# rehakvoj1/BIH-GPU-Raytracer

Measured on NVIDIA B200. Metric: Mrays/s, higher is better.
Workload: dtype f32

## Files before the change

### bih-gpu-raytracer_b200/csrc/api.cu

```cuda
#include "bihrt_internal.cuh"
#include <algorithm>
#include <cstdarg>
#include <cstdio>
#include <cstdlib>
#include <cstring>
#include <vector>

int bihrt_fail(bihrt_ctx* c, int code, const char* fmt, ...) {
    char buf[512];
    va_list ap;
    va_start(ap, fmt);
    vsnprintf(buf, sizeof buf, fmt, ap);
    va_end(ap);
    if (c) c->err = buf;
    return code;
}

#define ENTER(c) do { if (!(c)) return BIHRT_ERR_INVALID; BIHRT_CUDA((c), cudaSetDevice((c)->device)); } while (0)

static bool is_device_ptr(const void* p) {
    cudaPointerAttributes at;
    if (cudaPointerGetAttributes(&at, p) != cudaSuccess) { cudaGetLastError(); return false; }
    return at.type == cudaMemoryTypeDevice || at.type == cudaMemoryTypeManaged;
}
// ... 58 lines not shown
        size_t P = 256;
        while (P < (size_t)cap) P <<= 1;
        if ((rc = dev_alloc(c, &c->d_heaps, 4 * P))) return rc;
    }
    return BIHRT_OK;
}

extern "C" {

int bihrt_version(void) { return BIHRT_VERSION; }

int bihrt_create(bihrt_ctx** out, const bihrt_config* cfg) {
    if (!out) return BIHRT_ERR_INVALID;
    *out = nullptr;
    int ndev = 0;
    if (cudaGetDeviceCount(&ndev) != cudaSuccess || ndev == 0) { cudaGetLastError(); return BIHRT_ERR_CUDA; }
    bihrt_ctx* c = new (std::nothrow) bihrt_ctx();
    if (!c) return BIHRT_ERR_NOMEM;
    c->device = cfg ? cfg->device : 0;
    if (c->device < 0 || c->device >= ndev) { delete c; return BIHRT_ERR_INVALID; }
    cudaDeviceProp prop;
    if (cudaSetDevice(c->device) != cudaSuccess || cudaGetDeviceProperties(&prop, c->device) != cudaSuccess) { delete c; return BIHRT_ERR_CUDA; }
    if (prop.major < 10) { delete c; return BIHRT_ERR_CUDA; }
    c->sm_count = prop.multiProcessorCount;
    if (cudaStreamCreateWithFlags(&c->own_stream, cudaStreamNonBlocking) != cudaSuccess) { delete c; return BIHRT_ERR_CUDA; }
    c->stream = c->own_stream;
    cudaEventCreate(&c->ev0); cudaEventCreate(&c->ev1);
    int rc = 0;
    rc |= dev_alloc(c, &c->d_hist, 4096);
    rc |= dev_alloc(c, &c->d_scenebox_enc, 24);
    rc |= dev_alloc(c, &c->d_counters, 8);
    rc |= dev_alloc(c, &c->d_work, 1024);
    if (cudaHostAlloc((void**)&c->h_status, 64, cudaHostAllocMapped | cudaHostAllocPortable) != cudaSuccess ||
        cudaHostGetDevicePointer((void**)&c->d_status_map, c->h_status, 0) != cudaSuccess) { cudaGetLastError(); rc |= 1; }
    else *c->h_status = 0;
    if (rc) { bihrt_destroy(c); return BIHRT_ERR_NOMEM; }
    if (bihrt_build_setup(c) != BIHRT_OK) { bihrt_destroy(c); return BIHRT_ERR_CUDA; }
    *out = c;
    return BIHRT_OK;
}

void bihrt_destroy(bihrt_ctx* c) {
    if (!c) return;
    cudaSetDevice(c->device);
    cudaDeviceSynchronize();
    dev_free(&c->d_tri_in); dev_free(&c->d_blob);
    for (int i = 0; i < 2; i++) { dev_free(&c->d_keys[i]); dev_free(&c->d_vals[i]); }
    dev_free(&c->d_umc); dev_free(&c->d_first); dev_free(&c->d_hist); dev_free(&c->d_lookback);
    dev_free(&c->d_heaps); dev_free(&c->d_scenebox_enc);
    dev_free(&c->d_keys64[0]); dev_free(&c->d_keys64[1]); dev_free(&c->d_lookback_q);
    dev_free(&c->d_fb); dev_free(&c->d_counters); dev_free(&c->d_work);
    dev_free(&c->d_wtab); dev_free(&c->d_wscratch);
    for (auto& ts : c->tile_slots) { dev_free(&ts.cost); dev_free(&ts.order); }
    if (c->d_io) { cudaFree(c->d_io); c->d_io = nullptr; }
    for (int i = 0; i < 2; i++) { dev_free(&c->d_rs_keys[i]); dev_free(&c->d_rs_vals[i]); }
    dev_free(&c->d_rs_hist); dev_free(&c->d_rs_lookback); dev_free(&c->d_rs_hdr);
    if (c->h_status) { cudaFreeHost(c->h_status); c->h_status = nullptr; }
    if (c->ev0) cudaEventDestroy(c->ev0);
    if (c->ev1) cudaEventDestroy(c->ev1);
    if (c->build_graph_exec) cudaGraphExecDestroy(c->build_graph_exec);
    for (int i = 0; i < BIHRT_PROF_EVENTS; i++) if (c->prof_ev[i]) cudaEventDestroy(c->prof_ev[i]);
    if (c->own_stream) cudaStreamDestroy(c->own_stream);
    delete c;
}

const char* bihrt_last_error(const bihrt_ctx* c) { return c ? c->err.c_str() : "null context"; }

int bihrt_set_stream(bihrt_ctx* c, void* s) {
    ENTER(c);
    BIHRT_CUDA(c, cudaStreamSynchronize(c->stream));
    c->stream = (s == BIHRT_STREAM_OWN) ? c->own_stream : (cudaStream_t)s;
    return BIHRT_OK;
}

int bihrt_get_stream(bihrt_ctx* c, void** s) {
    if (!c || !s) return BIHRT_ERR_INVALID;
    *s = (void*)c->stream;
    return BIHRT_OK;
}

static int check_status(bihrt_ctx* c) {
    const uint32_t st = c->h_status ? *(volatile uint32_t*)c->h_status : 0u;
    if (st & 0x100u) return bihrt_fail(c, BIHRT_ERR_STATE, "the BIH in this context is a %s tree but the context traces %s trees: set the option morton_bits "
                                       "to the builder's value before adopting a replicated BIH", c->built_quality ? "parity" : "quality-mode", c->built_quality ? "quality-mode" : "parity");
    if (st) return bihrt_fail(c, BIHRT_ERR_INTERNAL, "device watchdog tripped during build (status %u): the BIH is invalid, rebuild", st);
    return BIHRT_OK;
}

int bihrt_sync(bihrt_ctx* c) {
    ENTER(c);
    BIHRT_CUDA(c, cudaStreamSynchronize(c->stream));
    return check_status(c);
}

int bihrt_set_option(bihrt_ctx* c, const char* name, int64_t v) {
    if (!c || !name) return BIHRT_ERR_INVALID;
    if (!strcmp(name, "trace_blocks_per_sm")) c->opt_trace_blocks_per_sm = (int)v;
    else if (!strcmp(name, "build_graph")) c->opt_build_graph = (int)v;
    else if (!strcmp(name, "morton_bits")) {
        if (v != 30 && v != 63) return bihrt_fail(c, BIHRT_ERR_INVALID, "morton_bits must be 30 (reference grid) or 63 (quality mode)");
        c->opt_morton_bits = (int)v;
        if (c->build_graph_exec) { cudaGraphExecDestroy(c->build_graph_exec); c->build_graph_exec = nullptr; }
    }
    else if (!strcmp(name, "leaf_cap")) {
        if (v < 1 || v > 64) return bihrt_fail(c, BIHRT_ERR_INVALID, "leaf_cap must be 1..64");
        c->opt_leaf_cap = (int)v;
        if (c->build_graph_exec) { cudaGraphExecDestroy(c->build_graph_exec); c->build_graph_exec = nullptr; }
    }
    else if (!strcmp(name, "debug_trip_watchdog")) {
        c->opt_debug_trip_watchdog = (int)v;
        if (c->build_graph_exec) { cudaGraphExecDestroy(c->build_graph_exec); c->build_graph_exec = nullptr; }
    }
    else if (!strcmp(name, "profile")) {
        BIHRT_CUDA(c, cudaSetDevice(c->device));
        c->opt_profile = (int)v;
        if (v) for (int i = 0; i < BIHRT_PROF_EVENTS; i++) if (!c->prof_ev[i]) cudaEventCreate(&c->prof_ev[i]);
    }
    else if (!strcmp(name, "trace_lane_groups")) c->opt_lane_groups = (int)v;
    else if (!strcmp(name, "trace_sort_rays")) c->opt_sort_rays = (int)v;
    else if (!strcmp(name, "trace_sm_queues")) c->opt_sm_queues = (int)v;
    else if (!strcmp(name, "trace_tile_sort_below")) c->opt_tile_sort_below = v;
    else if (!strcmp(name, "trace_tile_order")) { c->opt_tile_order = (int)v; for (auto& ts : c->tile_slots) ts.valid = false; }
    else if (!strcmp(name, "interleave_chunk")) c->opt_interleave_chunk = (int)std::max<int64_t>(1, std::min<int64_t>(1024, v));
    else return bihrt_fail(c, BIHRT_ERR_INVALID, "unknown option '%s'", name);
    return BIHRT_OK;
}

int bihrt_get_stat(bihrt_ctx* c, const char* name, int64_t* v) {
    if (!c || !name || !v) return BIHRT_ERR_INVALID;
    if (!strcmp(name, "kernel_launches")) *v = c->kernel_launches;
    else if (!strcmp(name, "sm_count")) *v = c->sm_count;
    else if (!strcmp(name, "trace_warp_node_steps") || !strcmp(name, "trace_warp_leaf_steps")) {
        unsigned long long h[2];
        BIHRT_CUDA(c, cudaSetDevice(c->device));
        BIHRT_CUDA(c, cudaMemcpyAsync(h, c->d_counters + 4, 16, cudaMemcpyDeviceToHost, c->stream));
        BIHRT_CUDA(c, cudaStreamSynchronize(c->stream));
        *v = (int64_t)h[name[11] == 'n' ? 0 : 1];
    }
    else if (!strncmp(name, "build_stage_ns_", 15)) {
        const int i = atoi(name + 15);
        if (!c->opt_profile || i < 0 || i + 1 >= c->prof_count) return bihrt_fail(c, BIHRT_ERR_STATE, "no profile for stage %d (set option profile=1 and build)", i);
        BIHRT_CUDA(c, cudaEventSynchronize(c->prof_ev[i + 1]));
        float ms = 0;
        BIHRT_CUDA(c, cudaEventElapsedTime(&ms, c->prof_ev[i], c->prof_ev[i + 1]));
        *v = (int64_t)(ms * 1e6f);
    }
    else return bihrt_fail(c, BIHRT_ERR_INVALID, "unknown stat '%s'", name);
    return BIHRT_OK;
}

static int upload_triangles(bihrt_ctx* c, const float* xyz9, int64_t n) {
    if (n > 0) {
        cudaMemcpyKind kind = is_device_ptr(xyz9) ? cudaMemcpyDeviceToDevice : cudaMemcpyHostToDevice;
        BIHRT_CUDA(c, cudaMemcpyAsync(c->d_tri_in, xyz9, (size_t)n * 36, kind, c->stream));
    }
    return BIHRT_OK;
}

int bihrt_scene_load_triangles(bihrt_ctx* c, const float* xyz9, int64_t n) {
    ENTER(c);
    if (n < 0 || (n > 0 && !xyz9)) return bihrt_fail(c, BIHRT_ERR_INVALID, "bad triangle array");
    if (n >= BIH_MAX_TRIS) return bihrt_fail(c, BIHRT_ERR_INVALID, "at most 2^29-1 triangles (29-bit child references)");
    int rc = ensure_capacity(c, n, true);
    if (rc) return rc;
    if (n != c->n) {
        bind_blob(c, std::max<int64_t>(n, 1));
        if (c->build_graph_exec) { cudaGraphExecDestroy(c->build_graph_exec); c->build_graph_exec = nullptr; }
    }
    c->n = n; c->have_scene = true; c->built = false; c->topology_valid = false;
    return upload_triangles(c, xyz9, n);
}

int bihrt_scene_update_vertices(bihrt_ctx* c, const float* xyz9, int64_t n) {
    ENTER(c);
    if (!c->have_scene || !c->d_tri_in) return bihrt_fail(c, BIHRT_ERR_STATE, "no scene loaded");
    if (n != c->n) return bihrt_fail(c, BIHRT_ERR_INVALID, "update must keep the triangle count (%lld != %lld)", (long long)n, (long long)c->n);
    c->built = false;
    return upload_triangles(c, xyz9, n);
}

int bihrt_scene_load_obj(bihrt_ctx* c, const char* path) {
    ENTER(c);
    if (!path) return BIHRT_ERR_INVALID;
    FILE* f = fopen(path, "r");
    if (!f) return bihrt_fail(c, BIHRT_ERR_IO, "cannot open '%s'", path);
    std::vector<float> verts, tris;
    std::vector<long> poly;
    char line[4096];
    int rc = BIHRT_OK;
    while (fgets(line, sizeof line, f)) {
// ... 715 lines not shown
```

### bih-gpu-raytracer_b200/csrc/bihrt_internal.cuh

```cuda
#pragma once
#include <cuda_runtime.h>
#include <stdint.h>
#include <string>
#include "../../include/bihrt.h"

struct __align__(16) BihNode {
    float    clip0;
    float    clip1;
    uint32_t ref_l;
    uint32_t ref_r;
    float    lbox[6];
    float    rbox[6];
};
static_assert(sizeof(BihNode) == 64, "node is one 64-byte record");
#define BIH_REF_LEAF  0x80000000u
#define BIH_REF_NODE(idx, axis) (((uint32_t)(idx) << 2) | (uint32_t)(axis))
#define BIH_REF_LEAFREF(slot)   (BIH_REF_LEAF | ((uint32_t)(slot) << 2))
#define BIH_REF_INDEX(ref)      (((ref) & 0x7FFFFFFFu) >> 2)
#define BIH_REF_AXIS(ref)       ((ref) & 3u)
#define BIH_MAX_TRIS  (1ll << 29)

struct __align__(16) BihTri {
    float    v0x, v0y, v0z, e1x;
    float    e1y, e1z, e2x, e2y;
// ... 18 lines not shown
#define BIHRT_PROF_EVENTS 16
struct bihrt_group;
struct bihrt_ctx {
    bihrt_group* group = nullptr; int group_rank = 0;
    int          device = 0;
    cudaStream_t stream = nullptr;
    cudaStream_t own_stream = nullptr;
    std::string  err;
    int          sm_count = 148;

    float*   d_tri_in = nullptr;
    int64_t  n = 0, cap_n = 0;
    bool     have_scene = false, built = false;
    bool     topology_valid = false;

    uint8_t* d_blob = nullptr;
    size_t   blob_cap = 0;
    BihHeader* d_hdr = nullptr;
    BihNode*   d_nodes = nullptr;
    BihTri*    d_tris = nullptr;

    uint32_t *d_keys[2] = {nullptr, nullptr}, *d_vals[2] = {nullptr, nullptr};
    uint64_t *d_keys64[2] = {nullptr, nullptr};
    uint32_t *d_lookback_q = nullptr; size_t lookback_q_words = 0;
    uint32_t *d_umc = nullptr;
    uint32_t *d_first = nullptr;
    uint32_t *d_hist = nullptr;
    uint32_t *d_lookback = nullptr;
    size_t    lookback_words = 0;
    float4   *d_heaps = nullptr;
    uint32_t *d_scenebox_enc = nullptr;

    uint32_t* d_fb = nullptr; int fb_w = 0, fb_h = 0; size_t fb_cap = 0;
    bool      fb_exported = false;
    uint32_t* h_status = nullptr;
    uint32_t* d_status_map = nullptr;
    void*     d_io = nullptr; size_t io_cap = 0;
    unsigned long long* d_counters = nullptr;
    uint32_t *d_rs_keys[2] = {nullptr, nullptr}, *d_rs_vals[2] = {nullptr, nullptr}, *d_rs_hist = nullptr, *d_rs_lookback = nullptr;
    BihHeader* d_rs_hdr = nullptr; size_t rs_cap = 0;
    int opt_sort_rays = 0;
    uint32_t* d_work = nullptr;
    struct TileKey {
        int mode = -1, w = 0, h = 0, gshift = 0, nsamp = 0, shard_index = 0, shard_count = 0, il_index = 0, il_count = 0, il_cshift = 0;
        int64_t nrays = 0; uint32_t ntiles = 0;
        bool operator==(const TileKey& o) const {
            return mode == o.mode && w == o.w && h == o.h && gshift == o.gshift && nsamp == o.nsamp && shard_index == o.shard_index &&
                   shard_count == o.shard_count && il_index == o.il_index && il_count == o.il_count && il_cshift == o.il_cshift &&
                   nrays == o.nrays && ntiles == o.ntiles;
        }
    };
    struct TileSlot { TileKey key; bool valid = false; uint32_t *cost = nullptr, *order = nullptr; size_t cap = 0; };
    TileSlot tile_slots[4]; int tile_next = 0;

    cudaEvent_t ev0 = nullptr, ev1 = nullptr;
    bool        build_timed = false;

    int opt_trace_blocks_per_sm = 0;
    int opt_lane_groups = -1;
    int opt_interleave_chunk = 8;
    int opt_tile_order = 1;
    int64_t opt_tile_sort_below = 4 << 20;
    int opt_sm_queues = -1;
    int64_t kernel_launches = 0;
    int opt_build_graph = 1;
    cudaGraphExec_t build_graph_exec = nullptr; int64_t build_graph_n = -1, build_graph_launches = 0;
    int opt_morton_bits = 30;
    int opt_leaf_cap = 4;
    bool built_quality = false;
    float*    d_wtab = nullptr; int64_t wtab_slots = 0;
    uint32_t* d_wscratch = nullptr;
    bool      wtab_valid = false;
    int opt_debug_trip_watchdog = 0;
    int opt_profile = 0;
    cudaEvent_t prof_ev[BIHRT_PROF_EVENTS] = {};
    int prof_count = 0;
};

int  bihrt_fail(bihrt_ctx* c, int code, const char* fmt, ...);
#define BIHRT_CUDA(c, call) do { cudaError_t e_ = (call); if (e_ != cudaSuccess) \
    return bihrt_fail((c), BIHRT_ERR_CUDA, "%s failed: %s (%s:%d)", #call, cudaGetErrorString(e_), __FILE__, __LINE__); } while (0)

#define H_HIST      0
#define H_TILECTR   2048
#define H_WORDS     2064
#define SORT_TILE   4096

int bihrt_sort_pairs_launch(bihrt_ctx* c, uint32_t* keys[2], uint32_t* vals[2], uint32_t n, int passes, uint32_t* hist, uint32_t* lookback, BihHeader* hdr);
int bihrt_build_launch(bihrt_ctx* c);
int bihrt_build_setup(bihrt_ctx* c);
int bihrt_build_launch_q(bihrt_ctx* c);
int bihrt_refit_launch(bihrt_ctx* c);
#define STACK_DEPTH_PARITY  32
#define STACK_DEPTH_QUALITY 96
struct TraceArgs {
    const BihHeader* hdr; const BihNode* nodes; const BihTri* tris;
    const bihrt_ray* rays; int64_t nrays;
    const uint32_t* perm;
    int any_hit; float tmax;
    float* out_t; int32_t* out_slot; int32_t* out_prim;
    bihrt_camera cam; int w, h, spp; uint64_t seed; uint32_t flags; int shard_index, shard_count;
    int s_begin, s_end;
    int il_index, il_count;
    int il_cshift;
    const uint32_t* tile_order;
    uint32_t* tile_cost;
    int gshift;
    uint32_t* fb;
    unsigned long long* counters; uint32_t* work;
    uint32_t* status_map;
    int queues;
    const bihrt_ray_interval* rays_iv;
    float* out_u; float* out_v; float* out_ng;
};
int bihrt_trace_launch(bihrt_ctx* c, const TraceArgs& a, int mode , bool counted);
int bihrt_resolve_launch(bihrt_ctx* c, uint32_t* fb, int npix, int spp);
int bihrt_tile_order_launch(bihrt_ctx* c, uint32_t* cost, uint32_t* order, uint32_t ntiles, bool full_sort);
struct ClosestArgs {
    const BihHeader* hdr; const BihNode* nodes; const BihTri* tris;
    const bihrt_point_query* pts; int64_t n;
    float* out_d2; float* out_u; float* out_v; int32_t* out_slot; int32_t* out_prim; float* out_q; float* out_ng;
    uint32_t* work;
    uint32_t* status_map;
};
int bihrt_closest_launch(bihrt_ctx* c, const ClosestArgs& a);
#define WTAB_FLOATS 32
#define WTAB_SCRATCH_WORDS(n) (4 * (size_t)(n) + 16)
struct WindingArgs {
    const BihHeader* hdr; const BihNode* nodes; const BihTri* tris;
    const float* wtab;
    const bihrt_point_query* pts; int64_t n;
    float b2;
    float* out_w;
    uint32_t* work;
    uint32_t* status_map;
};
int bihrt_winding_table_launch(bihrt_ctx* c);
int bihrt_winding_launch(bihrt_ctx* c, const WindingArgs& a);
int bihrt_ray_sort_launch(bihrt_ctx* c, const bihrt_ray* rays, int64_t n, const uint32_t** perm);
int bihrt_secondary_launch(bihrt_ctx* c, const float* t, const int32_t* slot, int64_t n, uint32_t* tile_cnt, unsigned long long* total,
                           const bihrt_camera& cam, int w, int h, int spp, uint64_t seed, uint32_t flags, int kind, const float light[3],
                           bihrt_ray* out_rays, int32_t* out_sample);

#ifdef __CUDACC__
__device__ __forceinline__ uint32_t enc_float(float f) {
    uint32_t u = __float_as_uint(f);
    return (u & 0x80000000u) ? ~u : (u | 0x80000000u);
}
__device__ __forceinline__ float dec_float(uint32_t u) {
    return __uint_as_float((u & 0x80000000u) ? (u & 0x7FFFFFFFu) : ~u);
}

__host__ __device__ __forceinline__ uint32_t bihrt_mix32(uint32_t x) {
    x ^= x >> 16; x *= 0x7feb352du; x ^= x >> 15; x *= 0x846ca68bu; x ^= x >> 16;
    return x;
}
__device__ __forceinline__ float bihrt_jitter(uint64_t seed, uint32_t pixel, uint32_t sample, uint32_t dim) {
    uint32_t h = bihrt_mix32((uint32_t)seed ^ bihrt_mix32(pixel + 0x9e3779b9u * (sample * 2u + dim + 1u)) ^ (uint32_t)(seed >> 32));
    return __fmul_rn((float)((h >> 8) + 1u), 1.0f / 16777216.0f);
// ... 10 lines not shown
```

### bih-gpu-raytracer_b200/csrc/trace.cu

```cuda
#include "bihrt_internal.cuh"
#include <float.h>

#define FULL 0xffffffffu
#define NONE 0xFFFFFFFFu
#define TRACE_THREADS 128
#define TRACE_MIN_BLOCKS 8
constexpr int NODE_STEPS = 4;

#define OCT_MIXED 8
#define BOX_EPS 2.384185791015625e-07f

#define DET_EPS __uint_as_float(0x358637beu)

struct Hit { float t; int slot; };

__device__ __forceinline__ float fmin3(float a, float b, float c) { float r; asm("min.f32 %0, %1, %2, %3;" : "=f"(r) : "f"(a), "f"(b), "f"(c)); return r; }
__device__ __forceinline__ float fmax3(float a, float b, float c) { float r; asm("max.f32 %0, %1, %2, %3;" : "=f"(r) : "f"(a), "f"(b), "f"(c)); return r; }

__device__ __forceinline__ uint32_t pack_colour(uint32_t hits, int samples) {
    const float fh = (float)hits, fm = (float)(samples - (int)hits), fs = (float)samples;
    float cr = __fdiv_rn(__fadd_rn(__fmul_rn(fh, 255.f), __fmul_rn(fm, 20.f)), fs);
    float cb = __fdiv_rn(__fmul_rn(fm, 40.f), fs);
    cr = fmaxf(0.f, fminf(255.f, cr));
    cb = fmaxf(0.f, fminf(255.f, cb));
// ... 10 lines not shown
__device__ __forceinline__ float mt_u(float ox, float oy, float oz, const float4& q0, float px, float py, float pz, float inv,
                                      float& tx, float& ty, float& tz) {
    tx = __fsub_rn(ox, q0.x); ty = __fsub_rn(oy, q0.y); tz = __fsub_rn(oz, q0.z);
    return __fmul_rn(__fadd_rn(__fadd_rn(__fmul_rn(tx, px), __fmul_rn(ty, py)), __fmul_rn(tz, pz)), inv);
}
__device__ __forceinline__ float mt_v(float dx, float dy, float dz, float e1x, float e1y, float e1z, float tx, float ty, float tz, float inv,
                                      float& qx, float& qy, float& qz) {
    qx = __fsub_rn(__fmul_rn(ty, e1z), __fmul_rn(e1y, tz));
    qy = __fsub_rn(__fmul_rn(tz, e1x), __fmul_rn(e1z, tx));
    qz = __fsub_rn(__fmul_rn(tx, e1y), __fmul_rn(e1x, ty));
    return __fmul_rn(__fadd_rn(__fadd_rn(__fmul_rn(dx, qx), __fmul_rn(dy, qy)), __fmul_rn(dz, qz)), inv);
}

template <bool COUNTED, bool FIRST, bool RANGE = false, bool TWO_SIDED = false>
__device__ __forceinline__ void test_leaf(const char* __restrict__ first_tri, float ox, float oy, float oz,
                                          float dx, float dy, float dz, Hit& h, uint32_t& ntris, uint32_t& wleaf,
                                          const float* tlo_p = nullptr) {
    const float4* p = reinterpret_cast<const float4*>(first_tri);
    for (;;) {
        const float4 q0 = __ldg(p), q1 = __ldg(p + 1), q2 = __ldg(p + 2);
        if (COUNTED) { ntris++; const uint32_t am = __activemask(); wleaf += ((threadIdx.x & 31) == __ffs(am) - 1); }
        const float e1x = q0.w, e1y = q1.x, e1z = q1.y, e2x = q1.z, e2y = q1.w, e2z = q2.x;
        float px, py, pz;
        const float det = mt_det(dx, dy, dz, e1x, e1y, e1z, e2x, e2y, e2z, px, py, pz);
        if (!((TWO_SIDED ? fabsf(det) : det) < DET_EPS)) {
            const float inv = __frcp_rn(det);
            float tx, ty, tz;
            const float u = mt_u(ox, oy, oz, q0, px, py, pz, inv, tx, ty, tz);
            if (!(u < 0.f || u > 1.f)) {
                float qx, qy, qz;
                const float v = mt_v(dx, dy, dz, e1x, e1y, e1z, tx, ty, tz, inv, qx, qy, qz);
                if (!(v < 0.f || __fadd_rn(u, v) > 1.f)) {
                    const float t = __fmul_rn(__fadd_rn(__fadd_rn(__fmul_rn(e2x, qx), __fmul_rn(e2y, qy)), __fmul_rn(e2z, qz)), inv);
                    if (t > (RANGE ? *tlo_p : 0.f) && t < h.t) {
                        h.t = t; h.slot = (int)__float_as_uint(q2.w);
                        if (FIRST) break;
                    }
                }
            }
        }
        if (__float_as_uint(q2.z) & 1u) break;
        p += 3;
    }
}

template <int MODE, bool COUNTED, bool Q>
__global__ void __launch_bounds__(TRACE_THREADS, TRACE_MIN_BLOCKS) k_trace(TraceArgs a) {
    constexpr int STACK_DEPTH = Q ? STACK_DEPTH_QUALITY : STACK_DEPTH_PARITY;
    constexpr bool COVER = MODE == 1;
    constexpr bool OCTS = MODE == 1;
    constexpr bool LIST = MODE == 0 || MODE == 3 || MODE == 4;
    constexpr bool RANGE = MODE == 3 || MODE == 4;
    constexpr bool TWO_SIDED = MODE == 4;
    __shared__ __align__(16) float s_ray[TRACE_THREADS * 10];
    const int lane = threadIdx.x & 31;
    const uint32_t lt = (1u << lane) - 1u;
    float* my_ray = s_ray + threadIdx.x * 10;
    const char* __restrict__ nodes_b = reinterpret_cast<const char*>(a.nodes);
    const char* __restrict__ tris_b = reinterpret_cast<const char*>(a.tris);
    const BihTri* __restrict__ tris = a.tris;
    const uint32_t nu = a.hdr->nu;
    if (a.hdr->status != 0) return;
    if ((a.hdr->quality != 0) != Q) {
        if (blockIdx.x == 0 && threadIdx.x == 0 && a.status_map) *a.status_map = 0x100u;
        return;
    }
    const float blo[3] = { a.hdr->lo[0], a.hdr->lo[1], a.hdr->lo[2] }, bhi[3] = { a.hdr->hi[0], a.hdr->hi[1], a.hdr->hi[2] };
    uint32_t nnodes = 0, ntris = 0, maxsp = 0;
    uint32_t wnode = 0, wleaf = 0;

    uint64_t total;
    int tx = 1;
    if (LIST) total = a.tile_cost ? (((uint64_t)a.nrays + 1023u) >> 10) << 10 : (uint64_t)a.nrays;
    else {
        tx = (a.w + 31) / 32;
        const int ty = (a.h + 31) / 32, T = tx * ty;
        const int my_tiles = T > a.shard_index ? (T - a.shard_index + a.shard_count - 1) / a.shard_count : 0;
        total = ((uint64_t)my_tiles * 1024u) << a.gshift;
    }
    const int gshift = LIST ? 0 : a.gshift;
    const int nsamp = LIST ? 1 : ((a.s_end - a.s_begin) >> gshift);
    uint32_t my_queue = 0;
    if (a.queues > 1) { asm("mov.u32 %0, %%smid;" : "=r"(my_queue)); my_queue %= (uint32_t)a.queues; }
    uint64_t pool_next = 0, pool_end = 0;
    long long unit_t0 = 0; uint32_t unit_tile = 0xFFFFFFFFu;
    bool exhausted = false;

    uint64_t item = ~0ull;
    int s = 0, s0 = 0;
    uint32_t hits = 0, pixel = 0, pxy = 0;
    float ix = 1.f, iy = 1.f, iz = 1.f, nx = 0.f, ny = 0.f, nz = 0.f, bpad = 0.f;
    uint32_t cur = NONE;
    float rMin = 0.f, pMin = 0.f, pMax = 0.f;
    Hit h; h.t = FLT_MAX; h.slot = -1;
    bool tracing = false;
    uint4 stack[STACK_DEPTH];
    int sp = 0;
#define STACK_RESET() do { sp = 0; } while (0)
#define STACK_PUSH(item) do { stack[sp] = (item); sp++; } while (0)
#define STACK_POP(e) do { sp--; (e) = stack[sp]; } while (0)
    const uint32_t root_ref = BIH_REF_NODE(0, a.hdr->root_axis);
    const bool direct = MODE == 1 && gshift > 0 && !(a.flags & BIHRT_RENDER_COUNTS);
    const uint32_t ray_smem = (uint32_t)__cvta_generic_to_shared(my_ray);

    for (;;) {
        const uint32_t busy = ~__ballot_sync(FULL, cur == NONE);
        if (busy == 0) {
            bool want_item = false, finishing = false;
            if (cur == NONE) {
                if (tracing) {
                    tracing = false;
                    if (MODE == 1) hits += (h.slot >= 0);
                    else if (RANGE) {
                        const bool hit = h.slot >= 0;
                        const bool rec = a.out_u || a.out_v || a.out_ng;
                        float u = 0.f, v = 0.f, gx = 0.f, gy = 0.f, gz = 0.f;
                        int32_t prim = -1;
                        if (hit && (rec || a.out_prim)) {
                            const float4* tq = reinterpret_cast<const float4*>(tris + h.slot);
                            const float4 q0 = __ldg(tq), q1 = __ldg(tq + 1), q2 = __ldg(tq + 2);
                            prim = (int32_t)__float_as_uint(q2.y);
                            if (rec) {
                                const float e1x = q0.w, e1y = q1.x, e1z = q1.y, e2x = q1.z, e2y = q1.w, e2z = q2.x;
                                const float2 dxy = *reinterpret_cast<const float2*>(my_ray + 6);
                                const float dx = dxy.x, dy = dxy.y, dz = my_ray[8];
                                float px, py, pz, tx, ty, tz, qx, qy, qz;
// ... 32 lines not shown
                if (finishing) {
                    const uint32_t same = __match_any_sync(fin, pixel);
                    const uint32_t sum = __reduce_add_sync(same, hits);
                    if (lane == __ffs(same) - 1) {
                        if (direct) a.fb[pixel] = pack_colour(sum, nsamp << gshift);
                        else if (sum) atomicAdd(&a.fb[pixel], sum);
                    }
                }
            }
            if (!LIST && a.tile_cost && unit_tile != 0xFFFFFFFFu) {
                if (lane == 0) atomicMax(a.tile_cost + unit_tile, (uint32_t)min((unsigned long long)(clock64() - unit_t0) >> 8, 0xFFFFFFFFull));
                unit_tile = 0xFFFFFFFFu;
            }
            uint32_t want = __ballot_sync(FULL, want_item);
            while (want && !exhausted) {
                if (pool_next >= pool_end) {
                    uint64_t base = ~0ull;
                    uint32_t got = 0;
                    if (lane == 0) {
                        const uint32_t ilc = (uint32_t)a.il_count, ili = (uint32_t)a.il_index, ics = (uint32_t)a.il_cshift;
                        if (a.queues <= 1) {
                            const uint64_t fetched = atomicAdd(a.work, 32u); got = 32;
                            const uint64_t lu = fetched >> 5;
                            base = ilc > 1 ? ((((lu >> ics) * ilc + ili) << ics) | (lu & ((1u << ics) - 1u))) << 5 : fetched;
                            if (base >= total) base = ~0ull;
                        } else {
                            const uint32_t tshift = 10 + gshift, ushift = 5 + gshift;
                            const uint64_t ntile = (total + ((1ull << tshift) - 1)) >> tshift;
                            for (uint32_t k = 0; k < (uint32_t)a.queues; k++) {
                                uint32_t q = my_queue + k; if (q >= (uint32_t)a.queues) q -= (uint32_t)a.queues;
                                if (q >= ntile) continue;
                                const uint32_t upt = (1u << ushift) / ilc;
                                const uint64_t units = ((ntile - q + a.queues - 1) / a.queues) * upt;
                                if (ld_relaxed(a.work + q) >= units) continue;
                                const uint32_t u = atomicAdd(a.work + q, 1u);
                                if (u >= units) continue;
                                const uint32_t lu = u % upt;
                                const uint64_t b = (((uint64_t)(u / upt) * a.queues + q) << tshift) + ((uint64_t)((((lu >> ics) * ilc + ili) << ics) | (lu & ((1u << ics) - 1u))) << 5);
                                if (b < total) { base = b; got = 32; break; }
                            }
                        }
                    }
                    base = __shfl_sync(FULL, base, 0);
                    got = __shfl_sync(FULL, got, 0);
                    if (LIST && a.tile_cost && unit_tile != 0xFFFFFFFFu) {
                        if (lane == 0) atomicMax(a.tile_cost + unit_tile, (uint32_t)min((unsigned long long)(clock64() - unit_t0) >> 8, 0xFFFFFFFFull));
                        unit_tile = 0xFFFFFFFFu;
                    }
                    if (base == ~0ull) { exhausted = true; break; }
                    pool_next = base;
                    pool_end = min(base + got, total);
                    if (a.tile_cost && unit_tile == 0xFFFFFFFFu) {
                        const uint32_t m = (uint32_t)(base >> (10 + gshift));
                        unit_tile = a.tile_order ? __ldg(a.tile_order + m) : m;
                        unit_t0 = clock64();
                    }
                }
                const uint64_t avail = pool_end - pool_next;
                const uint32_t rank = __popc(want & lt);
                const bool served = want_item && (uint64_t)rank < avail;
                if (served) {
                    item = pool_next + rank; s = 0; hits = 0; want_item = false;
                    if (LIST && a.tile_cost) {
                        const uint32_t mi = (uint32_t)(item >> 10);
                        const uint64_t ray = ((uint64_t)(a.tile_order ? __ldg(a.tile_order + mi) : mi) << 10) | (item & 1023u);
                        item = ray < (uint64_t)a.nrays ? ray : ~0ull;
                        if (item == ~0ull) want_item = true;
                    }
                    if (MODE == 0 && a.perm && item != ~0ull) item = __ldg(a.perm + item);
                    if (!LIST) {
                        const uint64_t pix = item >> gshift;
                        s0 = a.s_begin + (int)((uint32_t)item & ((1u << gshift) - 1u)) * nsamp;
                        const uint32_t mi = (uint32_t)(pix >> 10), q = (uint32_t)pix & 1023u;
                        const uint32_t m = a.tile_order ? __ldg(a.tile_order + mi) : mi;
                        const int tile = a.shard_index + (int)m * a.shard_count;
                        const int px = (tile % tx) * 32 + (int)((q >> 5) & 3u) * 8 + (int)(q & 7u);
                        const int py = (tile / tx) * 32 + (int)(q >> 7) * 4 + (int)((q >> 3) & 3u);
                        if (px < a.w && py < a.h) { pixel = (uint32_t)(py * a.w + px); pxy = (uint32_t)px | ((uint32_t)py << 16); }
                        else item = ~0ull;
                        if (item == ~0ull) want_item = true;
                    }
                }
                pool_next += min((uint64_t)__popc(want), avail);
                want = __ballot_sync(FULL, want_item);
            }
            if (cur == NONE && item != ~0ull) {
                float ox, oy, oz, dx, dy, dz;
                float tlo = 0.f, thi = FLT_MAX;
                bool live = true;
                if (RANGE) {
                    const float4* p = reinterpret_cast<const float4*>(a.rays_iv + item);
                    const float4 r0 = __ldg(p), r1 = __ldg(p + 1);
                    ox = r0.x; oy = r0.y; oz = r0.z; dx = r1.x; dy = r1.y; dz = r1.z;
                    tlo = fmaxf(r0.w, 0.f);
                    live = r0.w == r0.w && tlo < r1.w;
                    thi = fminf(r1.w, FLT_MAX);
                } else if (MODE == 0) {
                    const float* p = reinterpret_cast<const float*>(a.rays + item);
                    ox = __ldg(p); oy = __ldg(p + 1); oz = __ldg(p + 2); dx = __ldg(p + 3); dy = __ldg(p + 4); dz = __ldg(p + 5);
                } else {
                    const int px = (int)(pxy & 0xFFFFu), py = (int)(pxy >> 16);
                    const float ru = (a.flags & BIHRT_RENDER_JITTER) ? bihrt_jitter(a.seed, pixel, (uint32_t)(s0 + s), 0) : 0.5f;
                    const float rv = (a.flags & BIHRT_RENDER_JITTER) ? bihrt_jitter(a.seed, pixel, (uint32_t)(s0 + s), 1) : 0.5f;
                    const float uu = __fdiv_rn(__fadd_rn((float)px, ru), (float)a.w);
                    const float vv = __fdiv_rn(__fadd_rn((float)py, rv), (float)a.h);
                    ox = a.cam.origin[0]; oy = a.cam.origin[1]; oz = a.cam.origin[2];
                    dx = __fsub_rn(__fadd_rn(__fadd_rn(a.cam.lower_left[0], __fmul_rn(uu, a.cam.horizontal[0])), __fmul_rn(vv, a.cam.vertical[0])), ox);
                    dy = __fsub_rn(__fadd_rn(__fadd_rn(a.cam.lower_left[1], __fmul_rn(uu, a.cam.horizontal[1])), __fmul_rn(vv, a.cam.vertical[1])), oy);
                    dz = __fsub_rn(__fadd_rn(__fadd_rn(a.cam.lower_left[2], __fmul_rn(uu, a.cam.horizontal[2])), __fmul_rn(vv, a.cam.vertical[2])), oz);
                }
                ix = __frcp_rn(dx); iy = __frcp_rn(dy); iz = __frcp_rn(dz);
                nx = -__fmul_rn(ox, ix); ny = -__fmul_rn(oy, iy); nz = -__fmul_rn(oz, iz);
                bpad = __fmul_rn(BOX_EPS, fmaxf(fmaxf(fabsf(nx) <= FLT_MAX ? fabsf(nx) : 0.f, fabsf(ny) <= FLT_MAX ? fabsf(ny) : 0.f),
                                                fabsf(nz) <= FLT_MAX ? fabsf(nz) : 0.f));
                *reinterpret_cast<float2*>(my_ray) = make_float2(ox, ix); *reinterpret_cast<float2*>(my_ray + 2) = make_float2(oy, iy);
                *reinterpret_cast<float2*>(my_ray + 4) = make_float2(oz, iz); *reinterpret_cast<float2*>(my_ray + 6) = make_float2(dx, dy);
                my_ray[8] = dz;
                if (RANGE) my_ray[9] = tlo;
                h.t = RANGE ? thi : (MODE == 0 && a.any_hit) ? a.tmax : FLT_MAX; h.slot = -1; STACK_RESET(); tracing = true;
                bool in = nu > 0 && live;
                float tMin = __fmul_rn(__fsub_rn(ix < 0.f ? bhi[0] : blo[0], ox), ix);
                float tMax = __fmul_rn(__fsub_rn(ix < 0.f ? blo[0] : bhi[0], ox), ix);
                const float tymin = __fmul_rn(__fsub_rn(iy < 0.f ? bhi[1] : blo[1], oy), iy);
                const float tymax = __fmul_rn(__fsub_rn(iy < 0.f ? blo[1] : bhi[1], oy), iy);
                if ((tMin > tymax) || (tymin > tMax)) in = false;
                if (tymin > tMin) tMin = tymin;
                if (tymax < tMax) tMax = tymax;
                const float tzmin = __fmul_rn(__fsub_rn(iz < 0.f ? bhi[2] : blo[2], oz), iz);
                const float tzmax = __fmul_rn(__fsub_rn(iz < 0.f ? blo[2] : bhi[2], oz), iz);
                if ((tMin > tzmax) || (tzmin > tMax)) in = false;
// ... 137 lines not shown
        if constexpr (!OCTS) NODE_PHASE(OCT_MIXED);
        else switch (__float_as_int(my_ray[9])) {
            case 0: NODE_PHASE(0); break;
            case 1: NODE_PHASE(1); break;
            case 2: NODE_PHASE(2); break;
            case 3: NODE_PHASE(3); break;
            case 4: NODE_PHASE(4); break;
            case 5: NODE_PHASE(5); break;
            case 6: NODE_PHASE(6); break;
            case 7: NODE_PHASE(7); break;
            default: NODE_PHASE(OCT_MIXED); break;
        }
        if (cur + 1u > 0x80000000u) {
            const char* tp;
            asm("mad.wide.u32 %0, %1, 12, %2;" : "=l"(tp) : "r"(cur & 0x7FFFFFFCu), "l"(tris_b));
            const float2 dxy = *reinterpret_cast<const float2*>(my_ray + 6);
            test_leaf<COUNTED, COVER, RANGE, TWO_SIDED>(tp, my_ray[0], my_ray[2], my_ray[4], dxy.x, dxy.y, my_ray[8], h, ntris, wleaf, my_ray + 9);
            if (((LIST && a.any_hit) || COVER) && h.slot >= 0) { STACK_RESET(); cur = NONE; }
            else POP_VALID();
        }
#undef NODE_PHASE
#undef DEBUG_STACK_TRAP
#undef POP_VALID
#undef BOX_SLAB
#undef STACK_RESET
#undef STACK_PUSH
#undef STACK_POP
        __syncwarp();
    }

    if (COUNTED) {
#pragma unroll
        for (int o = 16; o > 0; o >>= 1) {
            nnodes += __shfl_xor_sync(FULL, nnodes, o);
            ntris += __shfl_xor_sync(FULL, ntris, o);
            maxsp = max(maxsp, __shfl_xor_sync(FULL, maxsp, o));
        }
        if (lane == 0) {
            atomicAdd(&a.counters[0], (unsigned long long)nnodes);
            atomicAdd(&a.counters[1], (unsigned long long)ntris);
            atomicMax(&a.counters[2], (unsigned long long)maxsp);
        }
        wnode = __reduce_add_sync(FULL, wnode); wleaf = __reduce_add_sync(FULL, wleaf);
        if (lane == 0) { atomicAdd(&a.counters[4], (unsigned long long)wnode); atomicAdd(&a.counters[5], (unsigned long long)wleaf); }
    }
}

__global__ void k_resolve(uint32_t* fb, int npix, int spp) {
    const int i = blockIdx.x * blockDim.x + threadIdx.x;
    if (i >= npix) return;
    fb[i] = pack_colour(fb[i], spp);
}

#define TILE_CLASSES 5
__device__ __forceinline__ int tile_class(uint32_t c, uint32_t mx) {
    int k = 0;
#pragma unroll
    for (int j = 1; j < TILE_CLASSES; j++) k += c < max(1u, mx >> j);
    return k;
}
__global__ void __launch_bounds__(1024) k_tile_order(uint32_t* __restrict__ cost, uint32_t* __restrict__ order, uint32_t ntiles) {
    __shared__ uint32_t s_w[TILE_CLASSES][32];
    __shared__ uint32_t s_max, s_base[TILE_CLASSES];
    const int lane = threadIdx.x & 31, w = threadIdx.x >> 5;
    const uint32_t per = (ntiles + 1023u) / 1024u, i0 = min(ntiles, threadIdx.x * per), i1 = min(ntiles, i0 + per);
    uint32_t mx = 0;
    for (uint32_t i = i0; i < i1; i++) mx = max(mx, cost[i]);
    mx = __reduce_max_sync(0xffffffffu, mx);
    if (lane == 0) s_w[0][w] = mx;
    __syncthreads();
    if (threadIdx.x == 0) { uint32_t m = 0; for (int k = 0; k < 32; k++) m = max(m, s_w[0][k]); s_max = m; }
    __syncthreads();
    mx = s_max;
    uint32_t cnt[TILE_CLASSES], inc[TILE_CLASSES];
#pragma unroll
    for (int k = 0; k < TILE_CLASSES; k++) cnt[k] = 0;
    for (uint32_t i = i0; i < i1; i++) {
        const int cl = tile_class(cost[i], mx);
#pragma unroll
        for (int k = 0; k < TILE_CLASSES; k++) cnt[k] += (cl == k);
    }
    __syncthreads();
#pragma unroll
    for (int k = 0; k < TILE_CLASSES; k++) {
        inc[k] = cnt[k];
#pragma unroll
        for (int o = 1; o < 32; o <<= 1) { const uint32_t t = __shfl_up_sync(0xffffffffu, inc[k], o); if (lane >= o) inc[k] += t; }
        if (lane == 31) s_w[k][w] = inc[k];
    }
    __syncthreads();
    if (threadIdx.x < TILE_CLASSES) {
        uint32_t run = 0;
        for (int j = 0; j < 32; j++) { const uint32_t x = s_w[threadIdx.x][j]; s_w[threadIdx.x][j] = run; run += x; }
        s_base[threadIdx.x] = run;
    }
    __syncthreads();
    if (threadIdx.x == 0) { uint32_t run = 0; for (int k = 0; k < TILE_CLASSES; k++) { const uint32_t x = s_base[k]; s_base[k] = run; run += x; } }
    __syncthreads();
    uint32_t pos[TILE_CLASSES];
#pragma unroll
    for (int k = 0; k < TILE_CLASSES; k++) pos[k] = s_base[k] + s_w[k][w] + inc[k] - cnt[k];
    for (uint32_t i = i0; i < i1; i++) {
        const int cl = tile_class(cost[i], mx);
#pragma unroll
        for (int k = 0; k < TILE_CLASSES; k++) if (cl == k) order[pos[k]++] = i;
    }
// ... 60 lines not shown

int bihrt_trace_launch(bihrt_ctx* c, const TraceArgs& a_in, int mode, bool counted) {
    TraceArgs a = a_in;
    const bool list = mode == 0 || mode == 3 || mode == 4;
    const int64_t rays = list ? a.nrays : (int64_t)a.w * a.h * (a.s_end - a.s_begin) / (a.shard_count > 0 ? a.shard_count : 1) / (a.il_count > 0 ? a.il_count : 1);
    const bool on = a.queues < 0 ? (rays >= (16ll << 20) && (list || a.gshift == 0)) : a.queues != 0;
    a.queues = on ? (c->sm_count < 1024 ? c->sm_count : 1024) : 1;
    uint32_t ntiles = 0;
    bihrt_ctx::TileKey key;
    if (!list) {
        const int tx = (a.w + 31) / 32, ty = (a.h + 31) / 32, T = tx * ty;
        const int mine = T > a.shard_index ? (T - a.shard_index + a.shard_count - 1) / a.shard_count : 0;
        if ((((uint64_t)mine * 1024u) << a.gshift) >= (1ull << 32) - (1ull << 24))
            return bihrt_fail(c, BIHRT_ERR_INVALID, "launch of %d tiles x 1024 pixels x %d lane groups exceeds the 32-bit work counter", mine, 1 << a.gshift);
    }
    const bool order_on = a.queues == 1 && (c->opt_tile_order > 1 || (c->opt_tile_order == 1 && rays >= (64ll << 10) && rays < (48ll << 20) && c->n >= 10000));
    if (order_on) {
        if (list) {
            if (a.nrays > 1024 && a.nrays <= (65536ll << 10)) { ntiles = (uint32_t)((a.nrays + 1023) >> 10); key.nrays = a.nrays; }
        } else {
            const int tx = (a.w + 31) / 32, ty = (a.h + 31) / 32, T = tx * ty;
            const int mine = T > a.shard_index ? (T - a.shard_index + a.shard_count - 1) / a.shard_count : 0;
            if (mine > 1 && mine <= 65536) ntiles = (uint32_t)mine;
            key.w = a.w; key.h = a.h; key.gshift = a.gshift; key.nsamp = a.s_end - a.s_begin; key.shard_index = a.shard_index;
            key.shard_count = a.shard_count; key.il_index = a.il_index; key.il_count = a.il_count; key.il_cshift = a.il_cshift;
        }
        key.mode = list ? mode : 1; key.ntiles = ntiles;
    }
    bihrt_ctx::TileSlot* slot = nullptr;
    if (ntiles) {
        for (auto& ts : c->tile_slots) if (ts.cap && ts.key == key) slot = &ts;
        if (!slot) {
            slot = &c->tile_slots[c->tile_next];
            c->tile_next = (c->tile_next + 1) % 4;
            slot->key = key; slot->valid = false;
        }
        if ((size_t)ntiles > slot->cap) {
            if (slot->cost) cudaFree(slot->cost);
            if (slot->order) cudaFree(slot->order);
            slot->cost = slot->order = nullptr; slot->cap = 0; slot->valid = false;
            if (cudaMalloc(&slot->cost, (size_t)ntiles * 4) != cudaSuccess || cudaMalloc(&slot->order, (size_t)ntiles * 4) != cudaSuccess) {
                cudaGetLastError();
                if (slot->cost) { cudaFree(slot->cost); slot->cost = nullptr; }
                slot = nullptr; ntiles = 0;
            } else slot->cap = ntiles;
        }
        if (slot) {
            if (!slot->valid) BIHRT_CUDA(c, cudaMemsetAsync(slot->cost, 0, (size_t)ntiles * 4, c->stream));
            a.tile_cost = slot->cost;
            a.tile_order = slot->valid ? slot->order : nullptr;
        }
    }
    a.status_map = c->d_status_map;
    int rc = c->built_quality ? launch_mode<true>(c, a, mode, counted) : launch_mode<false>(c, a, mode, counted);
    if (rc == BIHRT_OK && slot) {
        if ((rc = bihrt_tile_order_launch(c, slot->cost, slot->order, ntiles, rays < c->opt_tile_sort_below)) == BIHRT_OK) slot->valid = true;
    }
    return rc;
}
```

Measured before the change: 14680.

## Cull screen tiles whose ray frustum misses the scene box before tracing

```diff
diff --git a/bih-gpu-raytracer_b200/csrc/api.cu b/bih-gpu-raytracer_b200/csrc/api.cu
--- a/bih-gpu-raytracer_b200/csrc/api.cu
+++ b/bih-gpu-raytracer_b200/csrc/api.cu
@@ -134,6 +134,7 @@
     dev_free(&c->d_fb); dev_free(&c->d_counters); dev_free(&c->d_work);
     dev_free(&c->d_wtab); dev_free(&c->d_wscratch);
     for (auto& ts : c->tile_slots) { dev_free(&ts.cost); dev_free(&ts.order); }
+    dev_free(&c->d_cull);
     if (c->d_io) { cudaFree(c->d_io); c->d_io = nullptr; }
     for (int i = 0; i < 2; i++) { dev_free(&c->d_rs_keys[i]); dev_free(&c->d_rs_vals[i]); }
     dev_free(&c->d_rs_hist); dev_free(&c->d_rs_lookback); dev_free(&c->d_rs_hdr);
@@ -218,6 +219,15 @@
         BIHRT_CUDA(c, cudaMemcpyAsync(h, c->d_counters + 4, 16, cudaMemcpyDeviceToHost, c->stream));
         BIHRT_CUDA(c, cudaStreamSynchronize(c->stream));
         *v = (int64_t)h[name[11] == 'n' ? 0 : 1];
+    }
+    else if (!strcmp(name, "trace_tiles_culled")) {
+        uint32_t n = 0;
+        BIHRT_CUDA(c, cudaSetDevice(c->device));
+        if (c->d_cull) {
+            BIHRT_CUDA(c, cudaMemcpyAsync(&n, c->d_cull + 1, 4, cudaMemcpyDeviceToHost, c->stream));
+            BIHRT_CUDA(c, cudaStreamSynchronize(c->stream));
+        }
+        *v = (int64_t)n;
     }
     else if (!strncmp(name, "build_stage_ns_", 15)) {
         const int i = atoi(name + 15);
diff --git a/bih-gpu-raytracer_b200/csrc/bihrt_internal.cuh b/bih-gpu-raytracer_b200/csrc/bihrt_internal.cuh
--- a/bih-gpu-raytracer_b200/csrc/bihrt_internal.cuh
+++ b/bih-gpu-raytracer_b200/csrc/bihrt_internal.cuh
@@ -94,6 +94,7 @@
     };
     struct TileSlot { TileKey key; bool valid = false; uint32_t *cost = nullptr, *order = nullptr; size_t cap = 0; };
     TileSlot tile_slots[4]; int tile_next = 0;
+    uint32_t* d_cull = nullptr; size_t cull_cap = 0;
 
     cudaEvent_t ev0 = nullptr, ev1 = nullptr;
     bool        build_timed = false;
@@ -147,6 +148,7 @@
     int il_cshift;
     const uint32_t* tile_order;
     uint32_t* tile_cost;
+    const uint2* tile_list; const uint32_t* tile_live;
     int gshift;
     uint32_t* fb;
     unsigned long long* counters; uint32_t* work;
diff --git a/bih-gpu-raytracer_b200/csrc/trace.cu b/bih-gpu-raytracer_b200/csrc/trace.cu
--- a/bih-gpu-raytracer_b200/csrc/trace.cu
+++ b/bih-gpu-raytracer_b200/csrc/trace.cu
@@ -86,6 +86,7 @@
     constexpr bool LIST = MODE == 0 || MODE == 3 || MODE == 4;
     constexpr bool RANGE = MODE == 3 || MODE == 4;
     constexpr bool TWO_SIDED = MODE == 4;
+    constexpr bool CULL = MODE == 1;
     __shared__ __align__(16) float s_ray[TRACE_THREADS * 10];
     const int lane = threadIdx.x & 31;
     const uint32_t lt = (1u << lane) - 1u;
@@ -106,6 +107,7 @@
     uint64_t total;
     int tx = 1;
     if (LIST) total = a.tile_cost ? (((uint64_t)a.nrays + 1023u) >> 10) << 10 : (uint64_t)a.nrays;
+    else if (CULL) total = ((uint64_t)*a.tile_live * 1024u) << a.gshift;
     else {
         tx = (a.w + 31) / 32;
         const int ty = (a.h + 31) / 32, T = tx * ty;
@@ -244,7 +246,7 @@
                     pool_end = min(base + got, total);
                     if (a.tile_cost && unit_tile == 0xFFFFFFFFu) {
                         const uint32_t m = (uint32_t)(base >> (10 + gshift));
-                        unit_tile = a.tile_order ? __ldg(a.tile_order + m) : m;
+                        unit_tile = CULL ? __ldg(&a.tile_list[m].y) : a.tile_order ? __ldg(a.tile_order + m) : m;
                         unit_t0 = clock64();
                     }
                 }
@@ -264,10 +266,15 @@
                         const uint64_t pix = item >> gshift;
                         s0 = a.s_begin + (int)((uint32_t)item & ((1u << gshift) - 1u)) * nsamp;
                         const uint32_t mi = (uint32_t)(pix >> 10), q = (uint32_t)pix & 1023u;
-                        const uint32_t m = a.tile_order ? __ldg(a.tile_order + mi) : mi;
-                        const int tile = a.shard_index + (int)m * a.shard_count;
-                        const int px = (tile % tx) * 32 + (int)((q >> 5) & 3u) * 8 + (int)(q & 7u);
-                        const int py = (tile / tx) * 32 + (int)(q >> 7) * 4 + (int)((q >> 3) & 3u);
+                        int x0, y0;
+                        if (CULL) { const uint32_t e = __ldg(&a.tile_list[mi].x); x0 = (int)(e & 0xFFFFu); y0 = (int)(e >> 16); }
+                        else {
+                            const uint32_t m = a.tile_order ? __ldg(a.tile_order + mi) : mi;
+                            const int tile = a.shard_index + (int)m * a.shard_count;
+                            x0 = (tile % tx) * 32; y0 = (tile / tx) * 32;
+                        }
+                        const int px = x0 + (int)((q >> 5) & 3u) * 8 + (int)(q & 7u);
+                        const int py = y0 + (int)(q >> 7) * 4 + (int)((q >> 3) & 3u);
                         if (px < a.w && py < a.h) { pixel = (uint32_t)(py * a.w + px); pxy = (uint32_t)px | ((uint32_t)py << 16); }
                         else item = ~0ull;
                         if (item == ~0ull) want_item = true;
@@ -511,6 +518,120 @@
     fb[i] = pack_colour(fb[i], spp);
 }
 
+#define CULL_THREADS 128
+#define CULL_EPS 3.814697265625e-06
+#define CULL_DEAD 0xFFFFFFFFu
+__device__ bool tile_misses_box(const TraceArgs& a, const BihHeader* hdr, int x0, int y0) {
+    double o[3], ll[3], hz[3], vt[3], lo[3], hi[3];
+    for (int k = 0; k < 3; k++) {
+        o[k] = a.cam.origin[k]; ll[k] = a.cam.lower_left[k]; hz[k] = a.cam.horizontal[k]; vt[k] = a.cam.vertical[k];
+        lo[k] = hdr->lo[k]; hi[k] = hdr->hi[k];
+        if (!(fabs(o[k]) <= 1e18 && fabs(ll[k]) <= 1e18 && fabs(hz[k]) <= 1e18 && fabs(vt[k]) <= 1e18 &&
+              fabs(lo[k]) <= 1e18 && fabs(hi[k]) <= 1e18 && lo[k] <= hi[k])) return false;
+    }
+    const double u0 = (double)x0 / a.w, u1 = (double)(x0 + 32) / a.w, v0 = (double)y0 / a.h, v1 = (double)(y0 + 32) / a.h;
+    double c[3][4], dm[3], pn[3], pf[3], sg[3];
+    bool inside = true;
+    for (int k = 0; k < 3; k++) {
+        const double s = CULL_EPS * (fabs(lo[k] - o[k]) + fabs(hi[k] - o[k])) + 1e-30;
+        inside = inside && lo[k] - s <= o[k] && o[k] <= hi[k] + s;
+        const double b = ll[k] - o[k];
+        c[k][0] = b + u0 * hz[k] + v0 * vt[k]; c[k][1] = b + u1 * hz[k] + v0 * vt[k];
+        c[k][2] = b + u0 * hz[k] + v1 * vt[k]; c[k][3] = b + u1 * hz[k] + v1 * vt[k];
+        dm[k] = CULL_EPS * (fabs(ll[k]) + fabs(hz[k]) + fabs(vt[k]) + fabs(o[k]));
+        const double dlo = fmin(fmin(c[k][0], c[k][1]), fmin(c[k][2], c[k][3])) - dm[k];
+        const double dhi = fmax(fmax(c[k][0], c[k][1]), fmax(c[k][2], c[k][3])) + dm[k];
+        const double amin = fmin(fabs(dlo), fabs(dhi));
+        sg[k] = 0.0;
+        if ((dlo > 0.0 || dhi < 0.0) && amin >= 1e-30 && fmax(fabs(dlo), fabs(dhi)) <= 1e12) {
+            sg[k] = dlo > 0.0 ? 1.0 : -1.0;
+            pn[k] = (dlo > 0.0 ? lo[k] - s : hi[k] + s) - o[k]; pf[k] = (dlo > 0.0 ? hi[k] + s : lo[k] - s) - o[k];
+            if (fmax(fabs(pn[k]), fabs(pf[k])) > 1e30 * amin) return false;
+        } else if (o[k] == lo[k] || o[k] == hi[k]) return false;
+    }
+    if (inside) return false;
+    for (int j = 0; j < 3; j++) {
+        if (sg[j] == 0.0) continue;
+        if (pf[j] * sg[j] < 0.0) return true;
+        for (int i = 0; i < 3; i++) {
+            if (i == j || sg[i] == 0.0) continue;
+            const double sij = sg[i] * sg[j];
+            double m = DBL_MAX;
+            for (int q = 0; q < 4; q++) m = fmin(m, sij * (pn[i] * c[j][q] - pf[j] * c[i][q]));
+            if (m > fabs(pn[i]) * dm[j] + fabs(pf[j]) * dm[i]) return true;
+        }
+    }
+    return false;
+}
+
+__global__ void __launch_bounds__(CULL_THREADS) k_tile_cull(TraceArgs a, const uint32_t* __restrict__ order, uint32_t* cull,
+                                                           uint32_t ntiles, uint32_t quality) {
+    __shared__ uint32_t s_dead[CULL_THREADS], s_n;
+    __shared__ bool s_last;
+    uint2* ent = reinterpret_cast<uint2*>(cull + 4);
+    uint2* list = ent + ntiles;
+    const BihHeader* hdr = a.hdr;
+    const int tx = (a.w + 31) / 32;
+    if (threadIdx.x == 0) s_n = 0;
+    __syncthreads();
+    const uint32_t m = blockIdx.x * CULL_THREADS + threadIdx.x;
+    if (m < ntiles) {
+        const uint32_t t = order ? __ldg(order + m) : m;
+        const int tile = a.shard_index + (int)t * a.shard_count, x0 = (tile % tx) * 32, y0 = (tile / tx) * 32;
+        const bool dead = hdr->status == 0 && (hdr->quality != 0) == (quality != 0) && hdr->nu > 1 && tile_misses_box(a, hdr, x0, y0);
+        ent[m] = make_uint2(dead ? CULL_DEAD : (uint32_t)x0 | ((uint32_t)y0 << 16), t);
+        if (dead) s_dead[atomicAdd(&s_n, 1u)] = (uint32_t)tile;
+    }
+    __syncthreads();
+    const bool counts = a.flags & BIHRT_RENDER_COUNTS;
+    if (!(counts && a.gshift > 0)) {
+        const uint32_t value = counts ? 0u : pack_colour(0, a.s_end - a.s_begin);
+        const uint32_t ilc = (uint32_t)a.il_count, ili = (uint32_t)a.il_index, ics = (uint32_t)a.il_cshift;
+        for (uint32_t k = 0; k < s_n; k++) {
+            const int tile = (int)s_dead[k];
+            for (uint32_t q = threadIdx.x; q < 1024u; q += CULL_THREADS) {
+                const uint32_t unit = (q << a.gshift) >> 5;
+                if (ilc > 1 && ((unit >> ics) % ilc) != ili) continue;
+                const int px = (tile % tx) * 32 + (int)((q >> 5) & 3u) * 8 + (int)(q & 7u);
+                const int py = (tile / tx) * 32 + (int)(q >> 7) * 4 + (int)((q >> 3) & 3u);
+                if (px < a.w && py < a.h) a.fb[(size_t)py * a.w + px] = value;
+            }
+        }
+    }
+    __threadfence();
+    __syncthreads();
+    if (threadIdx.x == 0) s_last = atomicAdd(cull + 2, 1u) == gridDim.x - 1;
+    __syncthreads();
+    if (!s_last) return;
+    __threadfence();
+    constexpr uint32_t B = 16;
+    const uint32_t per = (ntiles + CULL_THREADS - 1) / CULL_THREADS, m0 = min(ntiles, threadIdx.x * per), m1 = min(ntiles, m0 + per);
+    uint32_t cnt = 0;
+    for (uint32_t b = m0; b < m1; b += B) {
+        uint32_t x[B];
+#pragma unroll
+        for (uint32_t k = 0; k < B; k++) x[k] = b + k < m1 ? __ldcg(&ent[b + k].x) : CULL_DEAD;
+#pragma unroll
+        for (uint32_t k = 0; k < B; k++) cnt += x[k] != CULL_DEAD;
+    }
+    const int lane = threadIdx.x & 31, w = threadIdx.x >> 5;
+    uint32_t inc = cnt;
+#pragma unroll
+    for (int o = 1; o < 32; o <<= 1) { const uint32_t t = __shfl_up_sync(0xffffffffu, inc, o); if (lane >= o) inc += t; }
+    if (lane == 31) s_dead[w] = inc;
+    __syncthreads();
+    uint32_t pos = inc - cnt, live = 0;
+    for (int k = 0; k < CULL_THREADS / 32; k++) { if (k < w) pos += s_dead[k]; live += s_dead[k]; }
+    for (uint32_t b = m0; b < m1; b += B) {
+        uint2 e[B];
+#pragma unroll
+        for (uint32_t k = 0; k < B; k++) e[k] = b + k < m1 ? __ldcg(ent + b + k) : make_uint2(CULL_DEAD, 0u);
+#pragma unroll
+        for (uint32_t k = 0; k < B; k++) if (e[k].x != CULL_DEAD) list[pos++] = e[k];
+    }
+    if (threadIdx.x == 0) { cull[0] = live; cull[1] = ntiles - live; cull[2] = 0; }
+}
+
 #define TILE_CLASSES 5
 __device__ __forceinline__ int tile_class(uint32_t c, uint32_t mx) {
     int k = 0;
@@ -677,6 +798,24 @@
         }
     }
     a.status_map = c->d_status_map;
+    if (mode == 1) {
+        const int tx = (a.w + 31) / 32, ty = (a.h + 31) / 32, T = tx * ty;
+        const uint32_t mine = T > a.shard_index ? (uint32_t)((T - a.shard_index + a.shard_count - 1) / a.shard_count) : 0u;
+        const size_t words = 4 + 4 * (size_t)mine;
+        if (words > c->cull_cap) {
+            if (c->d_cull) cudaFree(c->d_cull);
+            c->d_cull = nullptr; c->cull_cap = 0;
+            if (cudaMalloc(&c->d_cull, words * 4) != cudaSuccess) { cudaGetLastError(); return bihrt_fail(c, BIHRT_ERR_NOMEM, "cudaMalloc for the tile list failed"); }
+            c->cull_cap = words;
+            BIHRT_CUDA(c, cudaMemsetAsync(c->d_cull, 0, 16, c->stream));
+        }
+        k_tile_cull<<<mine ? (mine + CULL_THREADS - 1) / CULL_THREADS : 1, CULL_THREADS, 0, c->stream>>>(a, a.tile_order, c->d_cull, mine, c->built_quality ? 1u : 0u);
+        c->kernel_launches += 1;
+        BIHRT_CUDA(c, cudaGetLastError());
+        a.tile_order = nullptr;
+        a.tile_live = c->d_cull;
+        a.tile_list = reinterpret_cast<const uint2*>(c->d_cull + 4) + mine;
+    }
     int rc = c->built_quality ? launch_mode<true>(c, a, mode, counted) : launch_mode<false>(c, a, mode, counted);
     if (rc == BIHRT_OK && slot) {
         if ((rc = bihrt_tile_order_launch(c, slot->cost, slot->order, ntiles, rays < c->opt_tile_sort_below)) == BIHRT_OK) slot->valid = true;
```

After: 16220 (median of 6 runs). 10.5% higher.
